# uguryagmur/RealTimeObjectDetection

Hardware: AMD Instinct MI355X
Metric: frames/sec YOLOv3 608x608 bs=8 (Darknet.forward + write_results; 2 batches in flight, write_results_async on a second stream) (higher is better)
Workload: dtype f16x2-split (3 MFMA products, f32 accumulate); 1 GPU; YOLOv3 cfg 608x608 batch=8 per GPU, split-f16 MFMA conv + fused head + GPU NMS (BASELINE configs[2]); precision=f16s3, tiles=autotune (this run), parallelism=frame-shard x1, in_flight_batches=2, detections_last_step=1699, candidates_last_step=1914, f16_range_overflow=False

## Files before the change

### realtimeobjectdetection_amd/csrc/plan.cpp

```cpp
#include "plan.h"

#include <algorithm>
#include <cctype>
#include <cmath>
#include <cstdarg>
#include <cstdlib>
#include <cstring>
#include <map>
#include <mutex>
#include <sstream>

namespace rtod {

static thread_local std::string g_err;

void set_error(const char* fmt, ...) {
    char buf[1024];
    va_list ap;
    va_start(ap, fmt);
    vsnprintf(buf, sizeof(buf), fmt, ap);
    va_end(ap);
    g_err = buf;
}
const std::string& last_error_string() { return g_err; }
// ... 190 lines not shown
                L.w_off = woff;
                woff += (L.bn ? 4 : 1) * (int64_t)L.cout + (int64_t)L.cout * L.cin * L.size * L.size;
                conv_flops += 2ll * L.hout * L.wout * L.cout * L.cin * L.size * L.size;
                break;
            case LT_UPSAMPLE: L.cout = pc; L.hout = 2 * ph; L.wout = 2 * pw; break;
            case LT_MAXPOOL:
                L.cout = pc;
                if (L.pool_pad) { L.hout = (ph + 2 * L.pool_pad - L.size) / L.stride + 1; L.wout = (pw + 2 * L.pool_pad - L.size) / L.stride + 1; }
                else if (L.stride != 1) { L.hout = (ph - L.size) / L.stride + 1; L.wout = (pw - L.size) / L.stride + 1; }
                else { L.hout = ph; L.wout = pw; }
                if (L.hout < 1 || L.wout < 1) { set_error("cfg: layer %d: empty pool output", i); return RTOD_E_CFG; }
                break;
            case LT_SHORTCUT: {
                if (i < 1 || !src_ok(L.srcs[1])) { set_error("cfg: layer %d: shortcut source out of range", i); return RTOD_E_CFG; }
                const Layer& a = layers[L.srcs[0]]; const Layer& b = layers[L.srcs[1]];
                if (a.cout != b.cout || a.hout != b.hout || a.wout != b.wout) { set_error("cfg: layer %d: shortcut shape mismatch", i); return RTOD_E_CFG; }
                L.cout = a.cout; L.hout = a.hout; L.wout = a.wout;
                break;
            }
            case LT_ROUTE: {
                int c = 0;
                for (int s : L.srcs) {
                    if (!src_ok(s)) { set_error("cfg: layer %d: route source %d out of range", i, s); return RTOD_E_CFG; }
                    if (layers[s].hout != layers[L.srcs[0]].hout || layers[s].wout != layers[L.srcs[0]].wout) { set_error("cfg: layer %d: route spatial mismatch", i); return RTOD_E_CFG; }
                    c += layers[s].cout;
                }
                L.cout = c; L.cin = c; L.hout = layers[L.srcs[0]].hout; L.wout = layers[L.srcs[0]].wout;
                break;
            }
            case LT_YOLO: {
                if (i < 1) { set_error("cfg: yolo as first layer"); return RTOD_E_CFG; }
                const int A = (int)L.anchors.size();
                if (pc != A * (5 + L.classes)) { set_error("cfg: layer %d: head has %d channels, expected %d", i, pc, A * (5 + L.classes)); return RTOD_E_CFG; }
                if (ph > height || pw > width || height / (height / ph) != ph || width / (width / pw) != pw) {
                    set_error("cfg: layer %d: grid %dx%d does not divide input %dx%d", i, ph, pw, height, width); return RTOD_E_CFG;
                }
                if (height / ph != width / pw) {
                    set_error("cfg: layer %d: head grid %dx%d has stride %d along y but %d along x for input %dx%d (one integer stride on both axes is required)",
                              i, ph, pw, height / ph, width / pw, height, width);
                    return RTOD_E_CFG;
                }
                if (attrs && attrs != 5 + L.classes) { set_error("cfg: heads with different class counts"); return RTOD_E_CFG; }
                attrs = 5 + L.classes;
                L.cout = pc; L.hout = ph; L.wout = pw;
                L.row_offset = row_off; L.rows = ph * pw * A;
                row_off += L.rows;
                break;
            }
        }
        if (L.type == LT_YOLO) {
            prev_is_decoded = true;
            pc = layers[i - 1].cout; ph = layers[i - 1].hout; pw = layers[i - 1].wout;
        } else {
            prev_is_decoded = false;
            pc = L.cout; ph = L.hout; pw = L.wout;
        }
        if (L.type == LT_ROUTE || L.type == LT_SHORTCUT) prev_is_decoded = false;
    }
    total_rows = row_off;
    n_weight_floats = woff;
    if (total_rows == 0) { set_error("cfg: no yolo layer (the reference would return [])"); return RTOD_E_CFG; }
    return RTOD_OK;
}

static int resolve_alias(const std::vector<Layer>& layers, int i) {
    while (layers[i].alias_of >= 0) i = layers[i].alias_of;
    return i;
}

void Plan::reset_planning() {
    for (auto& L : layers) { L.fused_into = -1; L.fused_away = false; L.buf = -1; L.coff = 0; L.alias_of = -1; }
    bufs.clear(); launches.clear(); convs.clear(); input_buf = -1;
    tuned.clear(); tune_cache.clear(); tuning.clear();
}

int Plan::set_option(const char* name, int value) {
    if (!name) { set_error("set_option: null name"); return RTOD_E_ARG; }
    if (d_weights) { set_error("set_option: must be called before rtod_plan_load_weights"); return RTOD_E_STATE; }
    const std::string k(name);
    bool* flag = nullptr; int* num = nullptr;
    if (k == "fuse_pointwise") flag = &opt_fuse_pointwise;
    else if (k == "ring_kernel") flag = &opt_ring_kernel;
    else if (k == "pwd_kernel") flag = &opt_pwd_kernel;
    else if (k == "stem2_kernel") flag = &opt_stem2_kernel;
    else if (k == "k_slices") flag = &opt_k_slices;
    else if (k == "bn_batch_stats") {
        if (value && height != width) { set_error("set_option: bn_batch_stats is not supported on a rectangular plan (%dx%d)", height, width); return RTOD_E_ARG; }
        flag = &opt_bn_batch_stats;
    }
    else if (k == "k_slice_workgroups") flag = &opt_k_slice_workgroups;
    else if (k == "k_slices_split") flag = &opt_k_slices_split;
    else if (k == "patch_kernel") flag = &opt_patch_kernel;
    else if (k == "stem_kernel") flag = &opt_stem_kernel;
    else if (k == "band_kernel") flag = &opt_band_kernel;
    else if (k == "fuse_shortcut") flag = &opt_fuse_shortcut;
    else if (k == "fuse_decode") flag = &opt_fuse_decode;
    else if (k == "zero_copy_concat") flag = &opt_zero_copy_concat;
    else if (k == "narrow_cin") flag = &opt_narrow_cin;
    else if (k == "stem_pool") flag = &opt_stem_pool;
    else if (k == "fuse_stem_pool") flag = &opt_fuse_stem_pool;
    else if (k == "force_f16s3_variant") num = &opt_force_f16s3_variant;
    else if (k == "force_f32_variant") num = &opt_force_f32_variant;
    else { set_error("set_option: unknown option '%s'", name); return RTOD_E_ARG; }
    const bool old_flag = flag ? *flag : false; const int old_num = num ? *num : 0;
    if (flag) *flag = value != 0; else *num = value;
    return replan_or([&] { if (flag) *flag = old_flag; else *num = old_num; });
}

int Plan::replan_or(const std::function<void()>& restore) {
    reset_planning();
    int rc = plan_buffers();
    if (!rc && precision >= 1) rc = check_split_supported(precision);
    if (rc) {
        const std::string msg = last_error_string();
        restore();
        reset_planning();
        (void)plan_buffers();
        set_error("%s", msg.c_str());
    }
    return rc;
}

int Plan::set_precision(int mode) {
    const int old = precision;
    precision = mode;
    return replan_or([&] { precision = old; });
}

DecodeArgs Plan::decode_args(const Layer& Y) const {
    DecodeArgs d; d.enabled = 1; d.GH = Y.hout; d.GW = Y.wout; d.attrs = 5 + Y.classes; d.n_anchors = (int)Y.anchors.size();
    const int stride = height / Y.hout;
    d.stride = (float)stride;
    for (size_t a = 0; a < Y.anchors.size(); ++a) {
        d.aw[a] = (float)((double)Y.anchors[a].first / (double)stride);
        d.ah[a] = (float)((double)Y.anchors[a].second / (double)stride);
        if (Y.decode_v5) { d.aw[a] = (float)Y.anchors[a].first; d.ah[a] = (float)Y.anchors[a].second; }
    }
    d.v5 = Y.decode_v5 ? 1 : 0;
    d.img_stride = (int64_t)total_rows * attrs; d.head_off = (int64_t)Y.row_offset * attrs;
    return d;
}

int Plan::plan_buffers() {
    const int n = (int)layers.size();
    std::vector<std::vector<int>> cons(n);
    for (const auto& L : layers) {
        const int i = L.index;
        switch (L.type) {
            case LT_CONV: case LT_UPSAMPLE: case LT_MAXPOOL: case LT_YOLO: if (i > 0) cons[i - 1].push_back(i); break;
            case LT_SHORTCUT: case LT_ROUTE: for (int s : L.srcs) cons[s].push_back(i); break;
        }
    }
    for (auto& L : layers) {
        if (L.type == LT_ROUTE && L.srcs.size() == 1) L.alias_of = L.srcs[0];
        if (L.type == LT_YOLO) L.alias_of = L.index - 1;
    }
    for (auto& L : layers) {
        const int i = L.index;
        if (i == 0) continue;
        Layer& P = layers[i - 1];
        if (P.type != LT_CONV || P.fused_into >= 0 || cons[i - 1].size() != 1) continue;
        if (L.type == LT_SHORTCUT && L.srcs[1] != i - 1 && opt_fuse_shortcut) { P.fused_into = i; L.fused_away = true; }
        else if (L.type == LT_YOLO && cons[i].empty() && opt_fuse_decode) { P.fused_into = i; L.fused_away = true; }
    }
    auto materialised = [&](const Layer& L) {
        if (L.alias_of >= 0) return false;
// ... 360 lines not shown
                const double ps = std::ldexp(1.0, e);
                inv[o] = (float)(std::ldexp(1.0, -e) / (double)ACT_SCALE_F16S3);
                for (int c = 0; c < cin; ++c)
                    for (int ky = 0; ky < k; ++ky)
                        for (int kx = 0; kx < k; ++kx) {
                            const float v = (float)((double)p[(((int64_t)o * cin + c) * k + ky) * k + kx] * scale[o]);
                            const float vs = (float)((double)v * ps);
                            const uint16_t h = f32_to_f16_rn(vs);
                            const uint16_t l = f32_to_f16_rn(vs - f16_to_f32(h));
                            const int tap = ky * k + kx;
                            const int64_t idx = pc.narrow ? ((int64_t)(tap / 2) * pc.Npad + o) * 32 + (tap % 2) * 16 + c
                                                          : ((int64_t)((c / 32) * k * k + tap) * pc.Npad + o) * 32 + (c % 32);
                            wh[idx] = h; wl[idx] = l;
                        }
            }
        }
    }
    if (!d_weights) RTOD_HIP(hipMalloc((void**)&d_weights, sizeof(float) * (size_t)packed_floats));
    if (!d_arena) {
        RTOD_HIP(hipMalloc((void**)&d_arena, sizeof(float) * (size_t)arena_floats));
        if (precision == 2) RTOD_HIP(hipMemsetD16((hipDeviceptr_t)d_arena, 0x7E00, 2 * (size_t)arena_floats));
        else RTOD_HIP(hipMemset(d_arena, 0, sizeof(float) * (size_t)arena_floats));
    }
    if (opt_bn_batch_stats && !d_bn_stats && bn_stats_doubles > 0) {
        RTOD_HIP(hipMalloc((void**)&d_bn_stats, sizeof(double) * (size_t)bn_stats_doubles));
        RTOD_HIP(hipMemset(d_bn_stats, 0, sizeof(double) * (size_t)bn_stats_doubles));
        int maxn = 0;
        for (const auto& pc : convs) if (pc.stats_off >= 0) maxn = std::max(maxn, pc.Npad);
        bn_partial_count = (int64_t)bn_partial_doubles(maxn);
        RTOD_HIP(hipMalloc((void**)&d_bn_partial, sizeof(double) * (size_t)bn_partial_count));
    }
    if (!d_scratch) {
        bool any = false;
        for (const auto& pc : convs) any = any || (!pc.split && !pc.stem && pc.slice_chunks > 0) || (pc.split && pc.ks_chunks > 0);
        if (any) {
            scratch_floats = KS_SCRATCH_FLOATS;
            RTOD_HIP(hipMalloc((void**)&d_scratch, sizeof(float) * (size_t)scratch_floats));
        }
    }
    RTOD_HIP(hipMemcpy(d_weights, packed.data(), sizeof(float) * (size_t)packed_floats, hipMemcpyHostToDevice));
    RTOD_HIP(hipDeviceSynchronize());
    weights_loaded = true;
    return RTOD_OK;
}

int Plan::choose_variant(const Layer& L, int batch) const {
    if (opt_force_f32_variant >= 0 && opt_force_f32_variant < CV_COUNT) return opt_force_f32_variant;
    if (L.cout <= 32) return CV_128x32;
    if (L.cout <= 64) return CV_128x64;
    const int64_t M = (int64_t)batch * L.hout * L.wout;
    const int64_t big = ((M + 127) / 128) * ((L.cout + 127) / 128);
    return big >= 512 ? CV_128x128 : CV_64x64;
}

int Plan::f32_slice_mode(const Launch& l, int batch, int variant) const {
    const PackedConv& pc = convs[l.conv_slot];
    if (pc.split || pc.stem || pc.slice_chunks <= 0) return 0;
    const Layer& L = layers[l.layer];
    const ConvVariantInfo& vi = conv_variant_info(variant);
    const int64_t M = (int64_t)batch * L.hout * L.wout;
    const int64_t tiles = ((M + vi.bm - 1) / vi.bm) * ((L.cout + vi.bn - 1) / vi.bn);
    const int64_t S = (pc.Kpad / 32 + pc.slice_chunks - 1) / pc.slice_chunks;
    return (opt_k_slice_workgroups && d_scratch && tiles < 512 && S * M * pc.Npad <= scratch_floats) ? 2 : 1;
}

bool Plan::tile_legal(const Launch& l, int , int v) const {
    const TileRef t = family_of(v);
    if (!t || l.kind != LK_CONV || l.conv_slot < 0 || !convs[l.conv_slot].split) return false;
    const PackedConv& pc = convs[l.conv_slot];
    const Layer& L = layers[l.layer];
    if (precision == 2 && !t.f16()) return false;
    if (pc.narrow || t.is(TF_C16)) return pc.narrow && t.is(TF_C16);
    if (pc.ks_chunks > 0 || t.is(TF_KS)) return pc.ks_chunks > 0 && t.is(TF_KS);
    if (pc.band) return t.is(TF_BAND) && conv_band_mode_valid(t.mode, L.cin, L.hin, L.win);
    const bool hosts_pw = l.pw_guest >= 0 && pw_active(), plain = l.out_layer != -2 && !hosts_pw, same_map = L.hout == L.hin && L.wout == L.win;
    switch (t.fam->id) {
        case TF_GENERIC: return !(hosts_pw && t.fam->info(t.mode).bn < L.cout);
        case TF_BAND: return t.bandd_wide() && opt_band_kernel && plain && same_map && pc.Npad % 128 == 0 && pc.K == pc.Kpad &&
                             conv_bandd_wide_supported(L.size, L.stride, L.pad, pc.cin_p, L.win);
        case TF_RING: return !hosts_pw && L.act <= 1;
        case TF_PWD: return opt_pwd_kernel && plain && same_map && conv_pwd_supported(L.size, L.stride, L.pad, pc.cin_p);
        case TF_PATCH: return plain && L.act <= 1 && L.hout == L.hin && conv_patch_supported(L.size, L.stride, L.pad, L.cin, L.cout) &&
                              conv_patch_mode_valid(t.mode, L.cin, L.cout);
    }
    return false;
}

int Plan::default_tile(const Launch& l, int batch) const {
    const PackedConv& pc = convs[l.conv_slot];
    const Layer& L = layers[l.layer];
    const int64_t M = (int64_t)batch * L.hout * L.wout;
    if (pc.narrow) return tile_id(TF_C16, conv_c16_default_mode(L.cout, M));
    if (pc.ks_chunks > 0) return tile_id(TF_KS, ((M + 63) / 64) * ((L.cout + 63) / 64) < 512 ? 1 : 0);
    if (pc.band) {
        if (precision != 2) return tile_id(TF_BAND, conv_band_default_mode(L.cin, L.hin, L.win));
        const TileFamily& B = tile_family(TF_BAND);
        for (int m = 0; m < B.modes; ++m) if (tile_legal(l, batch, B.base + m)) return B.base + m;
        return B.base + B.f16_from;
    }
    const int64_t gn = (L.cout + 127) / 128;
    const int g = L.cout <= 64 ? HV_128x64 : ((M + 127) / 128) * gn >= 512 ? HV_128x128 : ((M + 63) / 64) * gn >= 512 ? HV_64x128 : HV_64x64;
    return tile_legal(l, batch, g) ? g : HV_128x128_8W;
}

int Plan::variant_for(const Launch& l, int batch) const {
    int want = opt_force_f16s3_variant;
    if (want < 0) {
        auto it = tuned.find(batch);
        const size_t idx = &l - &launches[0];
        if (it != tuned.end() && idx < it->second.size()) want = it->second[idx];
    }
    int v = want >= 0 && tile_legal(l, batch, want) ? want : default_tile(l, batch);
    if (family_of(v).ks_sched_b() && !(opt_k_slice_workgroups && ks_sched_b_fits(l, batch))) --v;
    return v;
}

std::vector<int> Plan::tile_candidates(const Launch& l, int batch) const {
    static const int kOrder[TF_COUNT] = {TF_GENERIC, TF_PATCH, TF_BAND, TF_PWD, TF_RING, TF_C16, TF_KS};
    const int cout = layers[l.layer].cout;
    const bool ks_b = opt_k_slice_workgroups && ks_sched_b_fits(l, batch);
    std::vector<int> cand;
    for (int f : kOrder) {
        if ((f == TF_RING && !opt_ring_kernel) || (f == TF_PATCH && !opt_patch_kernel)) continue;
        const TileFamily& F = tile_family(f);
        for (int m = 0; m < F.modes; ++m) {
            const int bn = F.info(m).bn;
            const bool too_wide = f == TF_GENERIC || f == TF_RING ? bn > 64 && bn > 2 * ((cout + 63) / 64 * 64)
                                : f == TF_PATCH ? bn > 64 && bn > cout
                                : f == TF_PWD ? bn > 128 && bn > (cout + 127) / 128 * 128 : false;
            if (too_wide || (family_of(F.base + m).ks_sched_b() && !ks_b) || !tile_legal(l, batch, F.base + m)) continue;
            cand.push_back(F.base + m);
        }
    }
    return cand;
}

int Plan::launch_split_variant(ConvArgs& a, const PackedConv& pc, int v, hipStream_t s) const {
    const TileRef t = family_of(v);
    if (!t) { set_error("variant %d is no split-f16 tile", v); return RTOD_E_STATE; }
    if (precision == 2 && !t.f16()) { set_error("variant %d has no plain-f16 instance", v); return RTOD_E_STATE; }
    if (pc.narrow != t.is(TF_C16)) {
        set_error(pc.narrow ? "variant %d requested for a narrow (Cin = 16) layer" : "narrow variant %d requested for a layer without tap-major weights", v);
        return RTOD_E_STATE;
    }
    if ((pc.ks_chunks > 0) != t.is(TF_KS)) {
        set_error(pc.ks_chunks > 0 ? "variant %d requested for a K-sliced layer" : "K-sliced variant %d requested for a layer that is not sliced", v);
        return RTOD_E_STATE;
    }
    if (pc.band != t.is(TF_BAND) && !(t.bandd_wide() && !pc.band)) {
        set_error(pc.band ? "variant %d requested for a band layer" : "band variant %d requested for a layer without band weights", v);
        return RTOD_E_STATE;
    }
    if (t.is(TF_KS)) {
        a.slice_chunks = pc.ks_chunks;
        a.partial = nullptr; a.partial_floats = 0;
        if (t.ks_sched_b()) { a.partial = d_scratch; a.partial_floats = scratch_floats; }
    }
    return t.fam->launch(a, t.mode, s);
}

int Plan::build_conv_args(const Launch& l, int batch, float* out, ConvArgs& a) const {
    const Layer& L = layers[l.layer];
    const PackedConv& pc = convs[l.conv_slot];
    const View in = view_of(l.in_layer);
    a.in = in.base; a.in_ldc = in.ldc; a.in_coff = in.coff;
    a.B = batch; a.Hi = L.hin; a.Wi = L.win; a.Cin = pc.cin_p;
    a.w = d_weights + pc.w_off; a.bias = d_weights + pc.b_off; a.K = pc.K; a.Kpad = pc.Kpad; a.Npad = pc.Npad;
    a.in_bytes = (unsigned)std::min<int64_t>((int64_t)batch * in.H * in.W * in.ldc * 4, 0xFFFFFFFFll);
    a.w_bytes = (unsigned)std::min<int64_t>((int64_t)pc.Npad * pc.Kpad * 2, 0xFFFFFFFFll);
    if (pc.split) {
        a.w_hi = reinterpret_cast<const _Float16*>(d_weights + pc.w_off);
        a.w_lo = reinterpret_cast<const _Float16*>(d_weights + pc.wl_off);
        a.inv_scale = d_weights + pc.s_off;
        a.f16 = precision == 2 ? 1 : 0;
    }
    a.kh = a.kw = L.size; a.stride = L.stride; a.pad = L.pad;
    a.Ho = L.hout; a.Wo = L.wout; a.Cout = L.cout; a.leaky = L.act;
    a.ovf = overflow_flag;
    if (in.C != pc.cin_p || in.H != L.hin || in.W != L.win) { set_error("forward: layer %d input view mismatch", l.layer); return RTOD_E_STATE; }
    if (l.out_layer == -2) { a.out = out; a.dec = l.dec; a.dec.train = train_decode; }
    else {
        const View o = view_of(l.out_layer);
        if (!o.base || o.C != L.cout || o.H != L.hout || o.W != L.wout) { set_error("forward: layer %d output view mismatch", l.layer); return RTOD_E_STATE; }
        a.out = o.base; a.out_ldc = o.ldc; a.out_coff = o.coff; a.out_split = o.split;
    }
    if (l.in2_layer >= 0) {
        const View r = view_of(l.in2_layer);
        if (!r.base || r.C != L.cout || r.H != L.hout || r.W != L.wout) { set_error("forward: layer %d residual view mismatch", l.layer); return RTOD_E_STATE; }
        a.res = r.base; a.res_ldc = r.ldc; a.res_coff = r.coff;
    }
    if (l.pw_guest >= 0 && pw_active()) {
        const Launch& g = launches[l.pw_guest];
        const Layer& G = layers[g.layer];
        const PackedConv& gc = convs[g.conv_slot];
        const View o = view_of(g.out_layer);
        if (!gc.split || gc.Kpad != L.cout || !o.base || !o.split || o.C != G.cout || o.H != L.hout || o.W != L.wout) { set_error("forward: layer %d fused pointwise mismatch", g.layer); return RTOD_E_STATE; }
        a.pw_wh = reinterpret_cast<const _Float16*>(d_weights + gc.w_off);
        a.pw_wl = reinterpret_cast<const _Float16*>(d_weights + gc.wl_off);
        a.pw_inv_scale = d_weights + gc.s_off; a.pw_bias = d_weights + gc.b_off;
        a.pw_out = o.base; a.pw_out_ldc = o.ldc; a.pw_out_coff = o.coff;
        a.pw_cout = G.cout; a.pw_k = L.cout; a.pw_leaky = G.act; a.pw_npad = gc.Npad;
    }
    return RTOD_OK;
}

static std::mutex g_tune_mutex;
static std::map<std::vector<int>, int> g_tune_memo;

int Plan::tune_launch(size_t li, ConvArgs& a, int batch, hipStream_t s) {
    const Launch& l = launches[li];
    const Layer& L = layers[l.layer];
    const bool pw = a.pw_wh != nullptr;
    const std::vector<int> key = {L.cin, L.cout, L.size, L.stride, L.hout, L.wout, l.in2_layer >= 0, l.out_layer == -2, pw ? a.pw_cout : 0,
                                  convs[l.conv_slot].band ? 1 : 0, opt_ring_kernel ? 1 : 0, opt_patch_kernel ? 1 : 0, opt_pwd_kernel ? 1 : 0, L.act,
                                  precision, L.hin, L.win, L.pad, convs[l.conv_slot].ks_chunks, opt_k_slice_workgroups ? 1 : 0};
    auto it = tune_cache.find(key);
    if (it != tune_cache.end()) { tuning[li] = it->second; return RTOD_OK; }
    std::vector<int> gkey = key; gkey.push_back(device); gkey.push_back(batch);
    {
        std::lock_guard<std::mutex> lock(g_tune_mutex);
        auto git = g_tune_memo.find(gkey);
        if (git != g_tune_memo.end()) { tuning[li] = git->second; tune_cache[key] = git->second; return RTOD_OK; }
    }
    hipEvent_t e0, e1;
    RTOD_HIP(hipEventCreate(&e0)); RTOD_HIP(hipEventCreate(&e1));
    const std::vector<int> cand = tile_candidates(l, batch);
    int best_v = variant_for(l, batch);
    int rc = RTOD_OK;
    auto time_variant = [&](int v, int reps, int per, float& out_ms) -> int {
        out_ms = 1e30f;
        for (int rep = 0; rep < reps; ++rep) {
            (void)hipEventRecord(e0, s);
            for (int r = 0; r < per; ++r) { const int q = launch_split_variant(a, convs[l.conv_slot], v, s); if (q) return q; }
            (void)hipEventRecord(e1, s);
            if (hipEventSynchronize(e1) != hipSuccess) return hip_fail(hipGetLastError(), "autotune sync");
            float ms = 0.f; (void)hipEventElapsedTime(&ms, e0, e1);
            out_ms = std::min(out_ms, ms / per);
        }
        return RTOD_OK;
    };
    std::vector<std::pair<float, int>> ranked;
    for (int v : cand) {
        rc = launch_split_variant(a, convs[l.conv_slot], v, s);
        if (rc) break;
        float ms; rc = time_variant(v, 3, 2, ms);
        if (rc) break;
        ranked.push_back({ms, v});
    }
    if (!rc && !ranked.empty()) {
        std::sort(ranked.begin(), ranked.end());
        const size_t top = std::min<size_t>(3, ranked.size());
        std::vector<float> fin(top, 1e30f);
        for (int round = 0; round < 5 && !rc; ++round)
            for (size_t t = 0; t < top && !rc; ++t) {
                float ms; rc = time_variant(ranked[t].second, 2, 4, ms);
                fin[t] = std::min(fin[t], ms);
            }
        if (!rc) best_v = ranked[std::min_element(fin.begin(), fin.end()) - fin.begin()].second;
    }
    (void)hipEventDestroy(e0); (void)hipEventDestroy(e1);
    if (rc) return rc;
    tuning[li] = best_v;
    tune_cache[key] = best_v;
    { std::lock_guard<std::mutex> lock(g_tune_mutex); g_tune_memo[gkey] = best_v; }
    return RTOD_OK;
}

int Plan::set_tiles(int batch, const int* variants, int count) {
    if (!variants || count != (int)launches.size() || batch <= 0 || batch > max_batch) { set_error("set_tiles: %d entries for %d launches, batch %d", count, (int)launches.size(), batch); return RTOD_E_ARG; }
    if (precision < 1) { set_error("set_tiles: split-f16 / f16 plans only"); return RTOD_E_STATE; }
    for (int i = 0; i < count; ++i) {
        const int v = variants[i];
        const Launch& l = launches[i];
        if (v < 0) continue;
        if (l.kind != LK_CONV || l.conv_slot < 0 || !convs[l.conv_slot].split) { set_error("set_tiles: launch %d is not a split-f16 convolution", i); return RTOD_E_ARG; }
        if (!tile_legal(l, batch, v)) { set_error("set_tiles: variant %d is not a valid tile of launch %d (layer %d)", v, i, l.layer); return RTOD_E_ARG; }
        if (family_of(v).ks_sched_b() && !ks_sched_b_fits(l, batch)) {
            set_error("set_tiles: variant %d (one workgroup per K slice) of launch %d (layer %d) needs more slice scratch than the plan has at batch %d", v, i, l.layer, batch);
            return RTOD_E_ARG;
        }
    }
    tuned[batch] = std::vector<int>(variants, variants + count);
    return RTOD_OK;
}

bool Plan::ks_sched_b_fits(const Launch& l, int batch) const {
    const PackedConv& pc = convs[l.conv_slot];
    if (pc.ks_chunks <= 0) return false;
    const Layer& L = layers[l.layer];
    const int64_t S = (pc.Kpad / 32 + pc.ks_chunks - 1) / pc.ks_chunks;
    return S * batch * L.hout * L.wout * pc.Npad <= KS_SCRATCH_FLOATS;
}
bool Plan::pw_active() const { return precision == 1 && opt_fuse_pointwise; }
bool Plan::stem_pool_fused() const { return precision >= 1 && stem_pool_pattern && !keep_all && convs[launches[0].conv_slot].stem16; }
bool Plan::stem2_active() const { return precision == 1 && opt_stem2_kernel && stem2_pattern && !keep_all && convs[launches[0].conv_slot].split; }

int Plan::forward(const float* x, int batch, float* out, hipStream_t s, float* launch_ms, bool tune) {
    if (!weights_loaded) { set_error("forward: load_weights has not been called"); return RTOD_E_STATE; }
// ... 189 lines not shown
```

### realtimeobjectdetection_amd/csrc/plan.h

```cpp
#pragma once
#include <functional>
#include <map>
#include <string>
#include <vector>

#include "rtod_internal.h"

namespace rtod {

enum LayerType { LT_CONV = 0, LT_SHORTCUT, LT_ROUTE, LT_UPSAMPLE, LT_MAXPOOL, LT_YOLO };
const char* layer_type_name(int t);

struct Layer {
    int index = 0;
    int type = LT_CONV;
    int cin = 0, cout = 0, hin = 0, win = 0, hout = 0, wout = 0;
    int size = 0, stride = 1, pad = 0;
    bool bn = false, leaky = false;
    int act = 0;
    bool nearest = false;
    bool decode_v5 = false;
    int pool_pad = 0;
    std::vector<int> srcs;
    std::vector<std::pair<int, int>> anchors;
    int classes = 0, row_offset = 0, rows = 0;
    int64_t w_off = 0;
    int fused_into = -1;
    bool fused_away = false;
    int buf = -1, coff = 0;
    int alias_of = -1;
};

struct Buffer {
    int C = 0, H = 0, W = 0;
    int first = 0, last = 0;
    int64_t floats_per_frame = 0;
    int64_t offset = 0;
};

enum LaunchKind { LK_CONV = 0, LK_PACK = 1, LK_UPSAMPLE = 2, LK_ADD = 3, LK_MAXPOOL = 4, LK_DECODE = 5, LK_COPY = 6, LK_STEM = 7 };

struct Launch {
    int kind = LK_CONV;
    int layer = 0;
    int in_layer = -1;
    int in2_layer = -1;
    int out_layer = -1;
    int out_buf = -1, out_coff = 0;
    int conv_slot = -1;
    DecodeArgs dec;
    int pw_guest = -1, pw_host = -1;
};

struct PackedConv {
    int layer = 0;
    int cin_p = 0, K = 0, Kpad = 0, Npad = 0;
    int64_t w_off = 0, b_off = 0;
    bool stem16 = false;
    bool stem = false;
    bool split = false;
    bool band = false;
    bool narrow = false;
    int64_t wl_off = 0, s_off = 0;
    int64_t stats_off = -1;
    int64_t bn_off = 0;
    int slice_chunks = 0;
    int ks_chunks = 0;
};

struct Plan {
    int height = 0, width = 0, max_batch = 0, device = 0;
    std::map<std::string, std::string> net_info;
    std::vector<Layer> layers;
    std::vector<Buffer> bufs;
    int input_buf = -1;
    std::vector<Launch> launches;
    std::vector<PackedConv> convs;
    int total_rows = 0, attrs = 0;
    int64_t n_weight_floats = 0, conv_flops = 0;
    int64_t arena_floats = 0, packed_floats = 0;
    float* d_arena = nullptr;
    float* d_weights = nullptr;
    double* d_bn_stats = nullptr;
    int64_t bn_stats_doubles = 0;
    double* d_bn_partial = nullptr;
    int64_t bn_partial_count = 0;
    float* d_scratch = nullptr;
    int64_t scratch_floats = 0;
    bool weights_loaded = false;
    int train_decode = 0;
    int precision = 0;
    bool keep_all = false;
    bool opt_fuse_pointwise = true;
    bool opt_stem_kernel = true;
    bool opt_band_kernel = true;
    bool opt_bn_batch_stats = false;
    bool opt_k_slices = true;
    bool opt_k_slice_workgroups = true;
    bool opt_k_slices_split = false;
    bool opt_stem2_kernel = true;
    bool opt_patch_kernel = true;
    bool opt_ring_kernel = true;
    bool opt_pwd_kernel = true;
    bool opt_fuse_shortcut = true;
    bool opt_fuse_decode = true;
    bool opt_zero_copy_concat = true;
    bool opt_narrow_cin = false;
    bool opt_stem_pool = false;
    bool opt_fuse_stem_pool = true;
    int opt_force_f16s3_variant = -1;
    int opt_force_f32_variant = -1;
    int32_t* overflow_flag = nullptr;
    std::vector<hipEvent_t> events;

    ~Plan();
    int parse(const std::string& cfg_text);
    int resolve_shapes();
    int plan_buffers();
    DecodeArgs decode_args(const Layer& yolo) const;
    int replan_or(const std::function<void()>& restore);
    void assign_arena();
    void layout_weights();
    bool uses_split(const Layer& L, int cin_p) const;
    int check_split_supported(int mode) const;
    int load_weights(const float* w, size_t n);
    int forward(const float* x, int batch, float* out, hipStream_t s, float* launch_ms, bool tune = false);
    int set_option(const char* name, int value);
    int set_precision(int mode);
    int set_tiles(int batch, const int* variants, int count);
    void reset_planning();
    View view_of(int layer) const;
    int choose_variant(const Layer& L, int batch) const;
    int build_conv_args(const Launch& l, int batch, float* out, ConvArgs& a) const;
    int tune_launch(size_t li, ConvArgs& a, int batch, hipStream_t s);
    std::vector<int> tuning;
    std::map<std::vector<int>, int> tune_cache;
    bool tile_legal(const Launch& l, int batch, int v) const;
    int default_tile(const Launch& l, int batch) const;
    int variant_for(const Launch& l, int batch) const;
    std::vector<int> tile_candidates(const Launch& l, int batch) const;
    int launch_split_variant(ConvArgs& a, const PackedConv& pc, int v, hipStream_t s) const;
    int f32_slice_mode(const Launch& l, int batch, int variant) const;
    bool ks_sched_b_fits(const Launch& l, int batch) const;
    bool pw_active() const;
    bool stem2_pattern = false;
    bool stem2_active() const;
    bool stem_pool_pattern = false;
    bool stem_pool_fused() const;
    std::map<int, std::vector<int>> tuned;
    std::string describe() const;
    void fill_launch_info(int idx, rtod_launch_info* o, int batch) const;
};

}
```

### realtimeobjectdetection_amd/csrc/rtod_internal.h

```cpp
#pragma once
#include <hip/hip_runtime.h>
#if defined(RTOD_STAMPS) && !defined(RTOD_DIAG)
#define RTOD_DIAG 1
#endif
#include <algorithm>
#include <atomic>
#include <cstdint>
#include <cstdio>
#include <string>
#include <vector>

#include "../../include/rtod.h"

namespace rtod {

void set_error(const char* fmt, ...);
int hip_fail(hipError_t e, const char* what);

#define RTOD_HIP(expr)                                              \
    do {                                                            \
        hipError_t _e = (expr);                                     \
        if (_e != hipSuccess) return ::rtod::hip_fail(_e, #expr);   \
    } while (0)

// ... 96 lines not shown
}
__device__ __forceinline__ __amdgpu_buffer_rsrc_t buffer_rsrc(const void* p, unsigned bytes) {
    return __builtin_amdgcn_make_buffer_rsrc(const_cast<void*>(p), 0, bytes, 0x00020000);
}
__device__ __forceinline__ int xcd_remap(int id, int n) {
    const int q = n >> 3, r = n & 7, xcd = id & 7;
    return (xcd < r ? xcd * (q + 1) : r * (q + 1) + (xcd - r) * q) + (id >> 3);
}
#endif

constexpr int EPI_F16 = 8;

enum ConvVariant { CV_128x128 = 0, CV_128x64 = 1, CV_64x64 = 2, CV_128x32 = 3, CV_COUNT };
struct ConvVariantInfo { int bm, bn; const char* name; };
const ConvVariantInfo& conv_variant_info(int v);
int conv_f32_kernel_name(int variant, char* buf, size_t len);
int launch_conv(const ConvArgs& a, int variant, hipStream_t s);
int conv_f32_slices(const ConvArgs& a);
enum ConvF16Variant { HV_128x128 = 0, HV_128x64 = 1, HV_64x64 = 2, HV_64x128 = 3, HV_256x128 = 4, HV_128x256 = 5, HV_128x128_8W = 6, HV_128x64_8W = 7, HV_256x128_16W = 8,
                      HV_192x128_8W = 9, HV_96x128_8W = 10, HV_192x128_12W = 11, HV_COUNT };
const ConvVariantInfo& conv_f16s3_variant_info(int v);
int conv_f16s3_kernel_name(int variant, int epi, char* buf, size_t len);
int launch_conv_f16s3(const ConvArgs& a, int variant, hipStream_t s);
bool conv_band_supported(int ksize, int stride, int pad, int cin, int w_in);
constexpr int BANDD_MODES = 9;
constexpr int BAND_LDS_MODES = 11;
constexpr int BAND_MODES = BAND_LDS_MODES + BANDD_MODES;
constexpr int BAND_K2_MODE0 = 7;
const ConvVariantInfo& conv_bandd_mode_info(int idx);
int conv_bandd_mode_kg(int idx);
constexpr int BANDD_WIDE_MODE = BAND_LDS_MODES + 7;
bool conv_bandd_wide_supported(int ksize, int stride, int pad, int cin, int w_in);
int conv_bandd_kernel_name(int idx, int epi, char* buf, size_t len);
int launch_conv_bandd_f16s3(const ConvArgs& a, int idx, hipStream_t s);
int conv_band_layer_kg(int cin, int h, int w);
bool conv_band_mode_valid(int mode, int cin, int h, int w);
int conv_band_default_mode(int cin, int h, int w);
const ConvVariantInfo& conv_band_mode_info(int mode);
int conv_band_kernel_name(int mode, int epi, char* buf, size_t len);
int launch_conv_band_f16s3(const ConvArgs& a, int mode, hipStream_t s);
constexpr int BAND_VARIANT_BASE = 50;
constexpr int RING_MODES = 8;
constexpr int RING_VARIANT_BASE = 70;
const ConvVariantInfo& conv_ring_mode_info(int mode);
int conv_ring_kernel_name(int mode, int epi, char* buf, size_t len);
int launch_conv_ring_f16s3(const ConvArgs& a, int mode, hipStream_t s);
constexpr int PWD_MODES = 11;
constexpr int PWD_VARIANT_BASE = 90;
bool conv_pwd_supported(int ksize, int stride, int pad, int cin);
const ConvVariantInfo& conv_pwd_mode_info(int mode);
int conv_pwd_kernel_name(int mode, int epi, char* buf, size_t len);
int launch_conv_pwd_f16s3(const ConvArgs& a, int mode, hipStream_t s);
constexpr int STEM2_VARIANT = 130;
bool conv_stem2_supported(int k0, int s0, int p0, int cin0, int cout0, int k1, int s1, int p1, int cout1, int pw_cout);
int conv_stem2_kernel_name(int pw, char* buf, size_t len);
int launch_conv_stem2_f16s3(const float* x, int B, int H, int W, const _Float16* w0h, const _Float16* w0l, const float* inv0, const float* bias0,
                            int leaky0, const ConvArgs& c1, hipStream_t s);
constexpr int PATCH_MODES = 5;
constexpr int PATCH_WRES_MODE = 4;
bool conv_patch_mode_valid(int mode, int cin, int cout);
constexpr int PATCH_VARIANT_BASE = 110;
bool conv_patch_supported(int ksize, int stride, int pad, int cin, int cout);
const ConvVariantInfo& conv_patch_mode_info(int mode);
int conv_patch_kernel_name(int mode, int epi, char* buf, size_t len);
int launch_conv_patch_f16s3(const ConvArgs& a, int mode, hipStream_t s);

constexpr int C16_MODES = 4;
constexpr int C16_VARIANT_BASE = 140;
constexpr bool conv_c16_supported(int cin) { return cin == 16; }
const ConvVariantInfo& conv_c16_mode_info(int mode);
int conv_c16_default_mode(int cout, int64_t m);
int conv_c16_kernel_name(int mode, int epi, char* buf, size_t len);
int launch_conv_c16_f16s3(const ConvArgs& a, int mode, hipStream_t s);

constexpr int KS_TILES = 3;
constexpr int KS_MODES = 2 * KS_TILES;
constexpr int KS_VARIANT_BASE = 150;
constexpr int64_t KS_SCRATCH_FLOATS = 8ll << 20;
const ConvVariantInfo& conv_ks_mode_info(int mode);
int conv_ks_slices(const ConvArgs& a);
int conv_ks_kernel_name(int mode, int epi, char* buf, size_t len);
int launch_conv_ks_f16s3(const ConvArgs& a, int mode, hipStream_t s);

enum TileFamilyId { TF_GENERIC = 0, TF_BAND, TF_RING, TF_PWD, TF_PATCH, TF_C16, TF_KS, TF_COUNT };
struct TileFamily {
    int id, base, modes;
    int f16_from;
    const ConvVariantInfo& (*info)(int mode);
    int (*kernel_name)(int mode, int epi, char* buf, size_t len);
    int (*launch)(const ConvArgs& a, int mode, hipStream_t s);
};
struct TileRef {
    const TileFamily* fam; int mode;
    explicit operator bool() const { return fam != nullptr; }
    bool is(int family) const { return fam && fam->id == family; }
    bool f16() const { return fam && mode >= fam->f16_from; }
    bool ks_sched_b() const { return is(TF_KS) && (mode & 1); }
    bool bandd_wide() const { return is(TF_BAND) && mode == BANDD_WIDE_MODE; }
};
TileRef family_of(int v);
const TileFamily& tile_family(int family);
inline int tile_id(int family, int mode) { return tile_family(family).base + mode; }

int launch_conv_stem(const float* x_nchw, const float* w, const float* bias, const View& out, int B, int H, int W,
                     int Ho, int Wo, int stride, int Cout, int leaky, hipStream_t s);
int launch_conv_stem_split(const float* x_nchw, const _Float16* wh, const _Float16* wl, const float* inv_scale, const float* bias,
                           const View& out, int B, int H, int W, int Ho, int Wo, int stride, int Cout, int leaky, int32_t* ovf, hipStream_t s);
bool conv_stem16_supported(int ksize, int stride, int pad, int cin, int cout, int act);
int launch_conv_stem16_f16s3(const float* x_nchw, const _Float16* wh, const _Float16* wl, const float* inv_scale, const float* bias,
                             const View& out, int B, int H, int W, int act, int pool, int32_t* ovf, hipStream_t s);
int launch_prep_image(const unsigned char* img, int h, int w, int bgr, int inp_dim, float* out, hipStream_t s);
int launch_prep_frames(const unsigned char* frames, int batch, int h, int w, int bgr, int out_h, int out_w, float* out, hipStream_t s);
int launch_pack_input(const float* x_nchw, int B, int C, int H, int W, float* out_nhwc, int Cp, hipStream_t s);
int launch_upsample2x(const View& in, const View& out, int B, hipStream_t s);
int launch_add(const View& a, const View& b, const View& out, int B, hipStream_t s);
int launch_maxpool(const View& in, const View& out, int B, int size, int stride, int pad, hipStream_t s);
int launch_upsample_nearest2x(const View& in, const View& out, int B, hipStream_t s);
int launch_bn_batch(const View& x, const View& y, const View* res, int B, double* stats, int sstride, const float* bn, int gstride, int act,
                    double* partial, int64_t partial_doubles, hipStream_t s);
size_t bn_partial_doubles(int max_channels);
struct BnUpdateEntry { float* running_mean; float* running_var; int64_t stats_off; double unbias; int sstride; int channels; };
constexpr int BN_UPDATE_MAX = 32;
struct BnUpdateTable { BnUpdateEntry e[BN_UPDATE_MAX]; };
int launch_bn_update_running(const BnUpdateEntry* entries, int n, const double* stats, double momentum, hipStream_t s);
int launch_copy(const View& in, const View& out, int B, hipStream_t s);
int launch_view_to_nchw(const View& in, int B, float* out_nchw, hipStream_t s);
int launch_decode(const float* raw, int64_t sb, int64_t sc, int64_t sy, int64_t sx, int B,
                  const DecodeArgs& d, float* out, hipStream_t s);
int launch_confidence_mask(const float* pred, int64_t rows, int attrs, float conf, float* out, hipStream_t s);
int launch_bbox_iou(const float* box1, const float* boxes, int k, int row_stride, float* iou, hipStream_t s);

size_t nms_workspace_bytes(int batch, int n);
int launch_write_results(const float* pred, int batch, int n, int num_class, float conf, float nms,
                         float* out, int cap, int32_t* counts, void* ws, size_t ws_bytes, hipStream_t s);
int launch_nms_class_offset(const float* pred, int batch, int n, int num_class, float conf, float iou_thr, float max_wh, int max_det,
                            float* out, int cap, int32_t* counts, void* ws, size_t ws_bytes, hipStream_t s);

}
```

### realtimeobjectdetection_amd/csrc/split_tiles.cpp

```cpp
#include "rtod_internal.h"

namespace rtod {

static const TileFamily kFamilies[TF_COUNT] = {
    {TF_GENERIC, 0, HV_COUNT, 0, conv_f16s3_variant_info, conv_f16s3_kernel_name, launch_conv_f16s3},
    {TF_BAND, BAND_VARIANT_BASE, BAND_MODES, BAND_LDS_MODES, conv_band_mode_info, conv_band_kernel_name, launch_conv_band_f16s3},
    {TF_RING, RING_VARIANT_BASE, RING_MODES, RING_MODES, conv_ring_mode_info, conv_ring_kernel_name, launch_conv_ring_f16s3},
    {TF_PWD, PWD_VARIANT_BASE, PWD_MODES, 0, conv_pwd_mode_info, conv_pwd_kernel_name, launch_conv_pwd_f16s3},
    {TF_PATCH, PATCH_VARIANT_BASE, PATCH_MODES, PATCH_MODES, conv_patch_mode_info, conv_patch_kernel_name, launch_conv_patch_f16s3},
    {TF_C16, C16_VARIANT_BASE, C16_MODES, 0, conv_c16_mode_info, conv_c16_kernel_name, launch_conv_c16_f16s3},
    {TF_KS, KS_VARIANT_BASE, KS_MODES, 0, conv_ks_mode_info, conv_ks_kernel_name, launch_conv_ks_f16s3},
};
static_assert(HV_COUNT <= BAND_VARIANT_BASE, "generic tile ids end where the band family's begin");
static_assert(BAND_VARIANT_BASE + BAND_MODES <= RING_VARIANT_BASE, "band tile ids end where the ring family's begin");
static_assert(RING_VARIANT_BASE + RING_MODES <= PWD_VARIANT_BASE, "ring tile ids end where the pwd family's begin");
static_assert(PWD_VARIANT_BASE + PWD_MODES <= PATCH_VARIANT_BASE, "pwd tile ids end where the patch family's begin");
static_assert(PATCH_VARIANT_BASE + PATCH_MODES <= STEM2_VARIANT && STEM2_VARIANT < C16_VARIANT_BASE, "the fused stem's reported id lies between the patch and narrow families");
static_assert(C16_VARIANT_BASE + C16_MODES <= KS_VARIANT_BASE, "narrow tile ids end where the K-sliced family's begin");

TileRef family_of(int v) {
    for (const TileFamily& f : kFamilies)
        if (v >= f.base && v < f.base + f.modes) return {&f, v - f.base};
    return {nullptr, 0};
}

const TileFamily& tile_family(int family) { return kFamilies[family]; }

}
```

Before: 2458 frames/s.

## Add direct-weight-register generic conv tile family to autotune candidates

Adds a new split-f16 conv kernel family (gbw) that stages only the activation panel through LDS while each wave streams its weight columns straight from global memory into registers, rotating them through several register sets. It is registered as a tile family, allowed for non-pointwise-hosting layers with unpadded K and Cin a multiple of 32, and offered to the autotuner. The aim is to cut LDS traffic and the barrier work of the weight operand on the generic conv layers. The cost is more register pressure and repeated global weight loads across workgroups, plus longer tuning time.

```diff
diff --git a/realtimeobjectdetection_amd/csrc/conv_gbw_f16s3.hip b/realtimeobjectdetection_amd/csrc/conv_gbw_f16s3.hip
--- /dev/null
+++ b/realtimeobjectdetection_amd/csrc/conv_gbw_f16s3.hip
@@ -0,0 +1,261 @@
+#include "conv_bandd_common.h"
+
+namespace rtod {
+
+template <int BM, int NW, int NB, int MINW, int EPI>
+__global__ __launch_bounds__(NW * 64, MINW)
+void conv_gbw_f16s3_kernel(const ConvArgs a, const int grid_m, const int grid_n) {
+    constexpr bool F16 = epi_f16(EPI);
+    constexpr int BN = NW * 32, NT = NW * 64, TM = BM / 16, TN = 2;
+    constexpr int RPP = NT / 4;
+    constexpr int A_SLOTS = (BM + RPP - 1) / RPP;
+    static_assert(BM % 16 == 0 && RPP % 16 == 0 && A_SLOTS >= 1 && A_SLOTS <= 2, "A stage shape");
+    static_assert(NB >= 2 && NB <= 4, "B sets");
+    constexpr int PANEL_A = BM * 64;
+    constexpr int STAGE = (F16 ? 1 : 2) * PANEL_A;
+    constexpr int LA = (F16 ? 1 : 2) * A_SLOTS, LB = F16 ? 2 : 4;
+    constexpr int WAIT = LA + (NB - 1) * LB;
+    constexpr bool DEC = epi_kind(EPI) == EPI_DECODE;
+    constexpr int RG = BM * BN * 4 <= 32768 ? BM : BM / 2;
+    constexpr int SMEM = DEC ? BM * BN * 4 : (2 * STAGE > RG * BN * 4 ? 2 * STAGE : RG * BN * 4);
+
+    extern __shared__ __attribute__((aligned(16))) unsigned char smem[];
+    const int nwg = grid_m * grid_n;
+    const int bid = xcd_remap(blockIdx.x, nwg);
+    const int bm = bid / grid_n, bn = bid - bm * grid_n;
+
+    const int tid = (int)threadIdx.x;
+    const int wave = __builtin_amdgcn_readfirstlane(tid >> 6), lane = tid & 63;
+    const int lr = lane & 15, lh = lane >> 4;
+    const int M = a.B * a.Ho * a.Wo;
+    const int c16 = tid & 3, row0 = tid >> 2;
+    const unsigned PS = (unsigned)a.in_ldc * 4u;
+    const unsigned lo_plane = (unsigned)a.in_ldc * 2u;
+
+    unsigned tapok[A_SLOTS];
+    unsigned pbase[A_SLOTS];
+#pragma unroll
+    for (int i = 0; i < A_SLOTS; ++i) {
+        const int m = bm * BM + row0 + i * RPP;
+        if (m < M && row0 + i * RPP < BM) {
+            const int hw = a.Ho * a.Wo;
+            const int b = m / hw, r = m - b * hw;
+            const int oy = r / a.Wo, ox = r - oy * a.Wo;
+            const int iy0 = oy * a.stride - a.pad, ix0 = ox * a.stride - a.pad;
+            pbase[i] = (unsigned)((b * a.Hi + iy0) * a.Wi + ix0) * PS + (unsigned)(a.in_coff + c16 * 8) * 2u;
+            unsigned ok = 0;
+            for (int ky = 0; ky < a.kh; ++ky)
+                for (int kx = 0; kx < a.kw; ++kx)
+                    if ((unsigned)(iy0 + ky) < (unsigned)a.Hi && (unsigned)(ix0 + kx) < (unsigned)a.Wi) ok |= 1u << (ky * a.kw + kx);
+            tapok[i] = ok;
+        } else {
+            tapok[i] = 0; pbase[i] = 0;
+        }
+    }
+
+    const __amdgpu_buffer_rsrc_t rs_a = buffer_rsrc(a.in, a.in_bytes);
+    const __amdgpu_buffer_rsrc_t rs_wh = buffer_rsrc(a.w_hi, a.w_bytes);
+    const __amdgpu_buffer_rsrc_t rs_wl = buffer_rsrc(a.w_lo, a.w_bytes);
+    const unsigned lds0 = (unsigned)(size_t)smem;
+
+    int ld_kc = 0, ld_c0 = 0, ld_ky = 0, ld_kx = 0;
+    const int nk = a.Kpad / HBK;
+
+    u32x4 Sh[2][A_SLOTS], Sl[2][A_SLOTS];
+    auto gload = [&](u32x4 (&sh)[A_SLOTS], u32x4 (&sl)[A_SLOTS]) __attribute__((always_inline)) {
+        const bool live = ld_kc < nk;
+        const unsigned tap_off = (unsigned)(ld_ky * a.Wi + ld_kx) * PS + (unsigned)ld_c0 * 2u;
+        const unsigned tap_bit = live ? 1u << (ld_ky * a.kw + ld_kx) : 0u;
+#pragma unroll
+        for (int i = 0; i < A_SLOTS; ++i) {
+            const unsigned vo = (tapok[i] & tap_bit) ? pbase[i] + tap_off : OOB;
+            sh[i] = buffer_load_b128(rs_a, vo, 0u);
+            if constexpr (!F16) sl[i] = buffer_load_b128(rs_a, vo, lo_plane);
+        }
+        ++ld_kc;
+        if (++ld_kx == a.kw) { ld_kx = 0; if (++ld_ky == a.kh) { ld_ky = 0; ld_c0 += HBK; } }
+    };
+    auto tie_stage = [&](u32x4 (&sh)[A_SLOTS], u32x4 (&sl)[A_SLOTS]) __attribute__((always_inline)) {
+        tie(sh);
+        if constexpr (!F16) tie(sl);
+    };
+    const int wr_swz = (c16 ^ ((row0 >> 1) & 3)) << 4;
+    auto lds_write = [&](const u32x4 (&sh)[A_SLOTS], const u32x4 (&sl)[A_SLOTS], int buf) __attribute__((always_inline)) {
+        unsigned char* st = smem + buf * STAGE;
+#pragma unroll
+        for (int i = 0; i < A_SLOTS; ++i) {
+            const int o = (row0 + i * RPP) * 64 + wr_swz;
+            if ((i + 1) * RPP <= BM || row0 + i * RPP < BM) {
+                *reinterpret_cast<u32x4*>(st + o) = sh[i];
+                if constexpr (!F16) *reinterpret_cast<u32x4*>(st + PANEL_A + o) = sl[i];
+            }
+        }
+    };
+
+    const int n0 = bn * BN + wave * 32;
+    const unsigned bvoff = n0 + lr < a.Npad ? (unsigned)((n0 + lr) * 32 + lh * 8) * 2u : OOB;
+    const unsigned wchunk = (unsigned)a.Npad * (HBK * 2);
+    u32x4 Bq[NB][TN][2];
+    auto load_b = [&](int t, u32x4 (&q)[TN][2]) __attribute__((always_inline)) {
+        const unsigned vo = t < nk ? bvoff : OOB;
+        const unsigned koff = (unsigned)__builtin_amdgcn_readfirstlane(t) * wchunk;
+        q[0][0] = buffer_load_b128(rs_wh, vo, koff);
+        if constexpr (!F16) q[0][1] = buffer_load_b128(rs_wl, vo, koff);
+        q[1][0] = buffer_load_b128<1024>(rs_wh, vo, koff);
+        if constexpr (!F16) q[1][1] = buffer_load_b128<1024>(rs_wl, vo, koff);
+    };
+
+    f32x4 acc[TM][TN];
+#pragma unroll
+    for (int i = 0; i < TM; ++i)
+#pragma unroll
+        for (int j = 0; j < TN; ++j)
+#pragma unroll
+            for (int e = 0; e < 4; ++e) acc[i][j][e] = 0.f;
+
+    typedef const f16x8 __attribute__((address_space(3))) lds_f16x8;
+    int a_off = (int)lds0 + lr * 64 + ((lh ^ ((lr >> 1) & 3)) << 4);
+    f16x8 Ah[2], Al[2];
+    auto read_unit = [&](int i, int buf, f16x8& h, f16x8& l) __attribute__((always_inline)) {
+        const int o = a_off + buf * STAGE + i * 1024;
+        h = *reinterpret_cast<lds_f16x8*>((unsigned)o);
+        if constexpr (!F16) l = *reinterpret_cast<lds_f16x8*>((unsigned)(o + PANEL_A));
+    };
+
+    gload(Sh[0], Sl[0]);
+    load_b(0, Bq[0]);
+    gload(Sh[1], Sl[1]);
+    if constexpr (NB == 3) load_b(1, Bq[1]);
+    vmcnt<WAIT>();
+    tie_stage(Sh[0], Sl[0]);
+    __builtin_amdgcn_sched_barrier(0);
+    lds_write(Sh[0], Sl[0], 0);
+    gload(Sh[0], Sl[0]);
+    __syncthreads();
+
+    auto step = [&](int t, auto q_c) __attribute__((always_inline)) {
+        constexpr int par = decltype(q_c)::value & 1, bs = decltype(q_c)::value % NB, nx = par ^ 1;
+        asm volatile("" : "+v"(a_off));
+        read_unit(0, par, Ah[0], Al[0]);
+        load_b(t + NB - 1, Bq[(bs + NB - 1) % NB]);
+        vmcnt<WAIT>();
+        tie_stage(Sh[nx], Sl[nx]);
+        tie_bset<F16>(Bq[bs]);
+        __builtin_amdgcn_sched_barrier(0);
+        lds_write(Sh[nx], Sl[nx], nx);
+        gload(Sh[nx], Sl[nx]);
+        __builtin_amdgcn_sched_barrier(0);
+#pragma unroll
+        for (int i = 0; i < TM; ++i) {
+            if (i + 1 < TM) read_unit(i + 1, par, Ah[(i + 1) % 2], Al[(i + 1) % 2]);
+            const f16x8 ah = Ah[i % 2], al = Al[i % 2];
+#pragma unroll
+            for (int j = 0; j < TN; ++j) {
+                const f16x8 bh = __builtin_bit_cast(f16x8, Bq[bs][j][0]);
+                if constexpr (F16) { acc[i][j] = __builtin_amdgcn_mfma_f32_16x16x32_f16(ah, bh, acc[i][j], 0, 0, 0); continue; }
+                const f16x8 bl = __builtin_bit_cast(f16x8, Bq[bs][j][1]);
+                acc[i][j] = __builtin_amdgcn_mfma_f32_16x16x32_f16(al, bh, acc[i][j], 0, 0, 0);
+                acc[i][j] = __builtin_amdgcn_mfma_f32_16x16x32_f16(ah, bl, acc[i][j], 0, 0, 0);
+                acc[i][j] = __builtin_amdgcn_mfma_f32_16x16x32_f16(ah, bh, acc[i][j], 0, 0, 0);
+            }
+            __builtin_amdgcn_sched_barrier(0);
+        }
+        __syncthreads();
+    };
+    constexpr int P = NB % 2 ? 2 * NB : NB;
+    auto run = [&](int t, auto q_c) __attribute__((always_inline)) {
+        step(t + decltype(q_c)::value, q_c);
+        return t + decltype(q_c)::value + 1 >= nk;
+    };
+    if constexpr (NB == 2) {
+#pragma unroll 1
+        for (int t = 0; t < nk; t += 2) {
+            step(t, std::integral_constant<int, 0>{});
+            step(t + 1, std::integral_constant<int, 1>{});
+        }
+    } else
+#pragma unroll 1
+    for (int t = 0;; t += P) {
+        if (run(t, std::integral_constant<int, 0>{})) break;
+        if (run(t, std::integral_constant<int, 1>{})) break;
+        if constexpr (P > 2) {
+            if (run(t, std::integral_constant<int, 2>{})) break;
+            if (run(t, std::integral_constant<int, 3>{})) break;
+        }
+        if constexpr (P > 4) {
+            if (run(t, std::integral_constant<int, 4>{})) break;
+            if (run(t, std::integral_constant<int, 5>{})) break;
+        }
+    }
+    vmcnt<0>();
+    tie_stage(Sh[0], Sl[0]); tie_stage(Sh[1], Sl[1]);
+#pragma unroll
+    for (int q = 0; q < NB; ++q) tie_bset<F16>(Bq[q]);
+    __builtin_amdgcn_sched_barrier(0);
+    int tid_e = tid;
+    asm volatile("" : "+v"(tid_e));
+    const int lr_e = tid_e & 15, lh_e = (tid_e >> 4) & 3;
+
+    if constexpr (DEC) conv_f16s3_epilogue<BM, BN, BM, 32, NT, EPI_DECODE, SMEM, 1, false, F16>(a, acc, smem, bm, bn, tid_e, 0, wave, lr_e, lh_e, M);
+    else bandd_epilogue<BM, BN, BM, 32, NT, RG, epi_kind(EPI) == EPI_SPLIT_RES, 1, F16>(a, acc, smem, bm, bn, tid_e, 0, wave, lr_e, lh_e, M, 0);
+}
+
+constexpr int gbw_lds_bytes(int bm, int bn, bool f16, bool dec) {
+    const int stages = 2 * (f16 ? 1 : 2) * bm * 64;
+    const int rg = bm * bn * 4 <= 32768 ? bm : bm / 2;
+    const int epi = dec ? bm * bn * 4 : rg * bn * 4;
+    return stages > epi ? stages : epi;
+}
+
+template <int BM, int NW, int NB, int MINW>
+static int launch_gbw(const ConvArgs& a, hipStream_t s) {
+    constexpr int BN = NW * 32, NT = NW * 64;
+    const int M = a.B * a.Ho * a.Wo;
+    const int gm = (M + BM - 1) / BM, gn = (a.Cout + BN - 1) / BN;
+    static_assert(gbw_lds_bytes(BM, BN, false, true) <= 64 * 1024, "dynamic LDS within the limit that needs no opt-in");
+    const bool fe = a.f16 != 0;
+    auto k_dec = fe ? conv_gbw_f16s3_kernel<BM, NW, NB, MINW, EPI_DECODE | EPI_F16> : conv_gbw_f16s3_kernel<BM, NW, NB, MINW, EPI_DECODE>;
+    auto k_res = fe ? conv_gbw_f16s3_kernel<BM, NW, NB, MINW, EPI_SPLIT_RES | EPI_F16> : conv_gbw_f16s3_kernel<BM, NW, NB, MINW, EPI_SPLIT_RES>;
+    auto k_plain = fe ? conv_gbw_f16s3_kernel<BM, NW, NB, MINW, EPI_SPLIT | EPI_F16> : conv_gbw_f16s3_kernel<BM, NW, NB, MINW, EPI_SPLIT>;
+    if (a.dec.enabled) hipLaunchKernelGGL(k_dec, dim3(gm * gn), dim3(NT), gbw_lds_bytes(BM, BN, fe, true), s, a, gm, gn);
+    else hipLaunchKernelGGL(a.res ? k_res : k_plain, dim3(gm * gn), dim3(NT), gbw_lds_bytes(BM, BN, fe, false), s, a, gm, gn);
+    return hip_fail(hipGetLastError(), "conv_gbw_f16s3 launch");
+}
+
+#define RTOD_GBW_TILES(X) \
+    X(0, 128, 4, 2, 3) X(1, 96, 4, 3, 3) X(2, 64, 4, 3, 4) X(3, 48, 4, 3, 4)
+
+#define RTOD_X_INFO(idx, bm, nw, nb, minw) {bm, nw * 32, "conv_gbw_f16s3<" #bm "x" #nw "w>"},
+static const ConvVariantInfo kGbwModes[GBW_MODES] = { RTOD_GBW_TILES(RTOD_X_INFO) };
+#undef RTOD_X_INFO
+const ConvVariantInfo& conv_gbw_mode_info(int idx) { return kGbwModes[idx < 0 || idx >= GBW_MODES ? 0 : idx]; }
+
+int conv_gbw_kernel_name(int idx, int epi, char* buf, size_t len) {
+#define RTOD_X_NAME(i, bm, nw, nb, minw) \
+    if (idx == i) return snprintf(buf, len, "void rtod::conv_gbw_f16s3_kernel<" #bm ", " #nw ", " #nb ", " #minw ", %d>(rtod::ConvArgs, int, int)", epi);
+    RTOD_GBW_TILES(RTOD_X_NAME)
+#undef RTOD_X_NAME
+    return -1;
+}
+
+int launch_conv_gbw_f16s3(const ConvArgs& a, int idx, hipStream_t s) {
+    if (int rc = check_split_conv_args(a, "launch_conv_gbw", true)) return rc;
+    if (a.Cin % HBK) { set_error("launch_conv_gbw: needs Cin %% 32 == 0 (Cin=%d)", a.Cin); return RTOD_E_ARG; }
+    if (a.K != a.Kpad || a.Kpad % HBK || a.K != a.kh * a.kw * a.Cin) { set_error("launch_conv_gbw: K = %d is not kh kw Cin without padding (Kpad=%d)", a.K, a.Kpad); return RTOD_E_ARG; }
+    if (a.kh * a.kw > 32) { set_error("launch_conv_gbw: kernel of %dx%d taps (at most 32)", a.kh, a.kw); return RTOD_E_ARG; }
+    if (a.pw_wh) { set_error("launch_conv_gbw: no hosted pointwise conv in this family"); return RTOD_E_ARG; }
+    if (a.in_ldc % 8 || a.in_coff % 8 || a.Npad % 128 || a.Npad < a.Cout) {
+        set_error("launch_conv_gbw: needs 8-channel aligned views and Npad %% 128 == 0 (ldc=%ld coff=%d Npad=%d)", (long)a.in_ldc, a.in_coff, a.Npad); return RTOD_E_ARG;
+    }
+    if (!a.dec.enabled && a.out_ldc <= 0) { set_error("launch_conv_gbw: bad output view"); return RTOD_E_ARG; }
+    if (a.B <= 0 || a.Ho <= 0 || a.Wo <= 0 || a.Cout <= 0) { set_error("launch_conv_gbw: empty shape"); return RTOD_E_ARG; }
+    switch (idx) {
+#define RTOD_X_CASE(i, bm, nw, nb, minw) case i: return launch_gbw<bm, nw, nb, minw>(a, s);
+        RTOD_GBW_TILES(RTOD_X_CASE)
+#undef RTOD_X_CASE
+    }
+    set_error("launch_conv_gbw: mode %d unsupported", idx);
+    return RTOD_E_ARG;
+}
+
+}
diff --git a/realtimeobjectdetection_amd/csrc/plan.cpp b/realtimeobjectdetection_amd/csrc/plan.cpp
--- a/realtimeobjectdetection_amd/csrc/plan.cpp
+++ b/realtimeobjectdetection_amd/csrc/plan.cpp
@@ -296,6 +296,7 @@
     if (k == "fuse_pointwise") flag = &opt_fuse_pointwise;
     else if (k == "ring_kernel") flag = &opt_ring_kernel;
     else if (k == "pwd_kernel") flag = &opt_pwd_kernel;
+    else if (k == "gbw_kernel") flag = &opt_gbw_kernel;
     else if (k == "stem2_kernel") flag = &opt_stem2_kernel;
     else if (k == "k_slices") flag = &opt_k_slices;
     else if (k == "bn_batch_stats") {
@@ -822,6 +823,7 @@
         case TF_PWD: return opt_pwd_kernel && plain && same_map && conv_pwd_supported(L.size, L.stride, L.pad, pc.cin_p);
         case TF_PATCH: return plain && L.act <= 1 && L.hout == L.hin && conv_patch_supported(L.size, L.stride, L.pad, L.cin, L.cout) &&
                               conv_patch_mode_valid(t.mode, L.cin, L.cout);
+        case TF_GBW: return opt_gbw_kernel && !hosts_pw && pc.K == pc.Kpad && pc.cin_p % 32 == 0;
     }
     return false;
 }
@@ -856,7 +858,7 @@
 }
 
 std::vector<int> Plan::tile_candidates(const Launch& l, int batch) const {
-    static const int kOrder[TF_COUNT] = {TF_GENERIC, TF_PATCH, TF_BAND, TF_PWD, TF_RING, TF_C16, TF_KS};
+    static const int kOrder[TF_COUNT] = {TF_GENERIC, TF_PATCH, TF_BAND, TF_PWD, TF_GBW, TF_RING, TF_C16, TF_KS};
     const int cout = layers[l.layer].cout;
     const bool ks_b = opt_k_slice_workgroups && ks_sched_b_fits(l, batch);
     std::vector<int> cand;
@@ -867,7 +869,7 @@
             const int bn = F.info(m).bn;
             const bool too_wide = f == TF_GENERIC || f == TF_RING ? bn > 64 && bn > 2 * ((cout + 63) / 64 * 64)
                                 : f == TF_PATCH ? bn > 64 && bn > cout
-                                : f == TF_PWD ? bn > 128 && bn > (cout + 127) / 128 * 128 : false;
+                                : f == TF_PWD || f == TF_GBW ? bn > 128 && bn > (cout + 127) / 128 * 128 : false;
             if (too_wide || (family_of(F.base + m).ks_sched_b() && !ks_b) || !tile_legal(l, batch, F.base + m)) continue;
             cand.push_back(F.base + m);
         }
@@ -953,7 +955,8 @@
     const bool pw = a.pw_wh != nullptr;
     const std::vector<int> key = {L.cin, L.cout, L.size, L.stride, L.hout, L.wout, l.in2_layer >= 0, l.out_layer == -2, pw ? a.pw_cout : 0,
                                   convs[l.conv_slot].band ? 1 : 0, opt_ring_kernel ? 1 : 0, opt_patch_kernel ? 1 : 0, opt_pwd_kernel ? 1 : 0, L.act,
-                                  precision, L.hin, L.win, L.pad, convs[l.conv_slot].ks_chunks, opt_k_slice_workgroups ? 1 : 0};
+                                  precision, L.hin, L.win, L.pad, convs[l.conv_slot].ks_chunks, opt_k_slice_workgroups ? 1 : 0,
+                                  opt_gbw_kernel ? 1 : 0, opt_band_kernel ? 1 : 0};
     auto it = tune_cache.find(key);
     if (it != tune_cache.end()) { tuning[li] = it->second; return RTOD_OK; }
     std::vector<int> gkey = key; gkey.push_back(device); gkey.push_back(batch);
diff --git a/realtimeobjectdetection_amd/csrc/plan.h b/realtimeobjectdetection_amd/csrc/plan.h
--- a/realtimeobjectdetection_amd/csrc/plan.h
+++ b/realtimeobjectdetection_amd/csrc/plan.h
@@ -102,6 +102,7 @@
     bool opt_patch_kernel = true;
     bool opt_ring_kernel = true;
     bool opt_pwd_kernel = true;
+    bool opt_gbw_kernel = true;
     bool opt_fuse_shortcut = true;
     bool opt_fuse_decode = true;
     bool opt_zero_copy_concat = true;
diff --git a/realtimeobjectdetection_amd/csrc/rtod_internal.h b/realtimeobjectdetection_amd/csrc/rtod_internal.h
--- a/realtimeobjectdetection_amd/csrc/rtod_internal.h
+++ b/realtimeobjectdetection_amd/csrc/rtod_internal.h
@@ -202,7 +202,13 @@
 int conv_ks_kernel_name(int mode, int epi, char* buf, size_t len);
 int launch_conv_ks_f16s3(const ConvArgs& a, int mode, hipStream_t s);
 
-enum TileFamilyId { TF_GENERIC = 0, TF_BAND, TF_RING, TF_PWD, TF_PATCH, TF_C16, TF_KS, TF_COUNT };
+constexpr int GBW_MODES = 4;
+constexpr int GBW_VARIANT_BASE = 170;
+const ConvVariantInfo& conv_gbw_mode_info(int mode);
+int conv_gbw_kernel_name(int mode, int epi, char* buf, size_t len);
+int launch_conv_gbw_f16s3(const ConvArgs& a, int mode, hipStream_t s);
+
+enum TileFamilyId { TF_GENERIC = 0, TF_BAND, TF_RING, TF_PWD, TF_PATCH, TF_C16, TF_KS, TF_GBW, TF_COUNT };
 struct TileFamily {
     int id, base, modes;
     int f16_from;
diff --git a/realtimeobjectdetection_amd/csrc/split_tiles.cpp b/realtimeobjectdetection_amd/csrc/split_tiles.cpp
--- a/realtimeobjectdetection_amd/csrc/split_tiles.cpp
+++ b/realtimeobjectdetection_amd/csrc/split_tiles.cpp
@@ -10,6 +10,7 @@
     {TF_PATCH, PATCH_VARIANT_BASE, PATCH_MODES, PATCH_MODES, conv_patch_mode_info, conv_patch_kernel_name, launch_conv_patch_f16s3},
     {TF_C16, C16_VARIANT_BASE, C16_MODES, 0, conv_c16_mode_info, conv_c16_kernel_name, launch_conv_c16_f16s3},
     {TF_KS, KS_VARIANT_BASE, KS_MODES, 0, conv_ks_mode_info, conv_ks_kernel_name, launch_conv_ks_f16s3},
+    {TF_GBW, GBW_VARIANT_BASE, GBW_MODES, 0, conv_gbw_mode_info, conv_gbw_kernel_name, launch_conv_gbw_f16s3},
 };
 static_assert(HV_COUNT <= BAND_VARIANT_BASE, "generic tile ids end where the band family's begin");
 static_assert(BAND_VARIANT_BASE + BAND_MODES <= RING_VARIANT_BASE, "band tile ids end where the ring family's begin");
@@ -17,6 +18,7 @@
 static_assert(PWD_VARIANT_BASE + PWD_MODES <= PATCH_VARIANT_BASE, "pwd tile ids end where the patch family's begin");
 static_assert(PATCH_VARIANT_BASE + PATCH_MODES <= STEM2_VARIANT && STEM2_VARIANT < C16_VARIANT_BASE, "the fused stem's reported id lies between the patch and narrow families");
 static_assert(C16_VARIANT_BASE + C16_MODES <= KS_VARIANT_BASE, "narrow tile ids end where the K-sliced family's begin");
+static_assert(KS_VARIANT_BASE + KS_MODES <= GBW_VARIANT_BASE, "K-sliced tile ids end where the direct-weight generic family's begin");
 
 TileRef family_of(int v) {
     for (const TileFamily& f : kFamilies)
```

After: 2457 frames/s. No clear change (-0.1%).
